# itailang/SampleNet

Hardware: NVIDIA H100
Metric: point-clouds/sec SampleNet fwd+Chamfer (B=32, N=1024->64) (higher is better)
Workload: dtype f32

## Files before the change

### samplenet_b200/csrc/conv_stack.cu

```cuda
#include "encoder_internal.cuh"
#include <cooperative_groups.h>
#include <string.h>

namespace snb {

constexpr int kCsMaxLayers = SNB200_MAX_CONV_LAYERS;
constexpr int kCsMaxSlicesPerCta = 32;
constexpr int kCsThreads = 512;
constexpr int kCsMaxPts = 128;
constexpr int kCsMinPts = 64;
constexpr int kCsNPT = kCsMaxPts / 4;
constexpr int kCsChunks = 4;
constexpr int kCsMaxSeg = 8;
constexpr int kCsLoPlane = kCsMaxPts * 128;
constexpr uint32_t kCsSlotBytes = 2u * kCsLoPlane;
constexpr int kCsWLd = 132;
constexpr uint32_t kCsWOff = kCsChunks * kCsSlotBytes;
constexpr uint32_t kCsAccOff = 2 * kCsSlotBytes;
constexpr size_t kCsSmemBytes = (size_t)kCsWOff + 128 * kCsWLd * sizeof(float) + 1024;

struct CsLayer {
    int c_in, c_out;
    const float *weight, *bias;
    const float *gamma, *beta, *run_mean, *run_var;
    float eps;
    int has_bn, relu;
    double *stats;
    float *zsave;
};

struct CsParams {
    const float *x; int layout;
    int b, n;
    long long total;
    int ppc, npt;
    int slots_per_cloud;
    int num_layers;
    CsLayer L[kCsMaxLayers];
    int training;
    double *mom;
    unsigned *barrier;
    float *tile_max, *tile_min;
    int fuse_head;
    HeadParams H;
    int self_clean;
    char *clean_ptr;
    unsigned clean_bytes;
    int slices_per_cta, num_slices;
    float *act[2];
    int act_ld;
    int head_rows;
};

__device__ __forceinline__ void cs_grid_arrive(unsigned *counter)
{
    asm volatile("red.release.gpu.global.add.u32 [%0], 1;" ::"l"(counter) : "memory");
}
__device__ __forceinline__ void cs_grid_wait(unsigned *counter, unsigned target)
{
    unsigned v, spin = 0;
    do {
        asm volatile("ld.acquire.gpu.global.u32 %0, [%1];" : "=r"(v) : "l"(counter) : "memory");
        if (++spin > (1u << 26)) __trap();
    } while (v < target);
}
__device__ __forceinline__ void cs_grid_barrier(unsigned *counter, unsigned target)
{
    __syncthreads();
    if (threadIdx.x == 0) {
        __threadfence();
        atomicAdd(counter, 1u);
        unsigned v, spin = 0;
        do {
            asm volatile("ld.acquire.gpu.global.u32 %0, [%1];" : "=r"(v) : "l"(counter) : "memory");
            if (++spin > (1u << 26)) __trap();
        } while (v < target);
    }
    __syncthreads();
}

__device__ __forceinline__ void cs_xchg_store(float *p, float v)
{
    unsigned u = __float_as_uint(v);
    if (u == 0u) u = 0x80000000u;
    asm volatile("st.volatile.global.u32 [%0], %1;" ::"l"(p), "r"(u) : "memory");
}
__device__ __forceinline__ unsigned cs_xchg_load1(const float *p)
{
    unsigned v;
    asm volatile("ld.volatile.global.u32 %0, [%1];" : "=r"(v) : "l"(p) : "memory");
    return v;
}
__device__ __forceinline__ uint4 cs_xchg_load4(const float *p)
{
    uint4 v;
    asm volatile("ld.volatile.global.v4.u32 {%0, %1, %2, %3}, [%4];" : "=r"(v.x), "=r"(v.y), "=r"(v.z), "=r"(v.w) : "l"(p) : "memory");
    return v;
}

__device__ __forceinline__ void cs_head_stage_weights(const HeadLayer &L, int cb, int nch, float *s_wh, int tid)
{
    const int c_in = L.c_in;
    if ((c_in & 3) == 0) {
        const int q4 = c_in >> 2, total = 8 * q4;
        for (int e0 = tid; e0 < total; e0 += kCsThreads * 4) {
            float4 v[4];
#pragma unroll
            for (int u = 0; u < 4; u++) {
                const int e = e0 + u * kCsThreads;
                const int jr = e / q4, kq = e - jr * q4;
                v[u] = (e < total && jr < nch) ? __ldg(reinterpret_cast<const float4 *>(L.weight + (size_t)(cb + jr) * c_in) + kq) : make_float4(0, 0, 0, 0);
            }
#pragma unroll
            for (int u = 0; u < 4; u++) {
                const int e = e0 + u * kCsThreads;
                if (e < total) *reinterpret_cast<float4 *>(s_wh + (size_t)e * 4) = v[u];
            }
        }
    } else {
        for (int e = tid; e < 8 * c_in; e += kCsThreads) {
            const int jr = e / c_in, k = e - jr * c_in;
            s_wh[e] = (jr < nch) ? __ldg(L.weight + (size_t)(cb + jr) * c_in + k) : 0.f;
        }
    }
}


__device__ __forceinline__ float cs_ld_now(const float *p)
{
    float v;
    asm volatile("ld.global.cg.f32 %0, [%1];" : "=f"(v) : "l"(p) : "memory");
    return v;
}

template <int KR>
__device__ __forceinline__ void cs_head_dot(const float *x, const float *w, int c_in, float (&a4)[4])
{
    float xr[KR];
#pragma unroll
    for (int i = 0; i < KR; i++) xr[i] = x[i];
#pragma unroll
    for (int i = 0; i < KR; i += 4) {
#pragma unroll
        for (int j = 0; j < 4; j++) {
            const float4 wv = *reinterpret_cast<const float4 *>(w + j * c_in + i);
            a4[j] = fmaf(xr[i + 3], wv.w, fmaf(xr[i + 2], wv.z, fmaf(xr[i + 1], wv.y, fmaf(xr[i], wv.x, a4[j]))));
        }
    }
}

__device__ __forceinline__ double cs_stat(const double *base, int c2, int idx, int spread)
{
    return __ldcg(spread ? base + c2 + (size_t)idx * kStatStride : base + idx);
}

constexpr unsigned long long kFxCountOne = 1ull << 56, kFxFieldMask = kFxCountOne - 1;
constexpr long long kFxSumOffset = 1ll << 47;
__device__ __forceinline__ unsigned long long *cs_fx_line(double *stats, int C, int idx)
{
    return reinterpret_cast<unsigned long long *>(stats + 2 * C + (size_t)idx * kStatStride);
}
__device__ __forceinline__ void cs_fx_add(unsigned long long *p, unsigned long long v)
{
    asm volatile("red.relaxed.gpu.global.add.u64 [%0], %1;" ::"l"(p), "l"(v) : "memory");
}
__device__ __forceinline__ unsigned long long cs_fx_load(const unsigned long long *p)
{
    unsigned long long v;
    asm volatile("ld.relaxed.gpu.global.u64 %0, [%1];" : "=l"(v) : "l"(p) : "memory");
    return v;
}
__device__ __forceinline__ bool cs_fx_contribute(double *stats, int C, int ch, float sum, float sumsq)
{
    const bool ok = fabsf(sum) < 8388608.f && sumsq < 274877906944.f;
    if (!ok) { sum = 0.f; sumsq = 0.f; }
    const long long ps = __double2ll_rn((double)sum * 16777216.0) + kFxSumOffset;
    const double qd = (double)sumsq, qh = floor(qd * 512.0);
    const long long hi = (long long)qh, lo = __double2ll_rn((qd - qh * (1.0 / 512.0)) * 281474976710656.0);
    unsigned long long *la = cs_fx_line(stats, C, ch), *lb = cs_fx_line(stats, C, C + ch);
    cs_fx_add(la, kFxCountOne + (unsigned long long)ps);
    cs_fx_add(lb, kFxCountOne + (unsigned long long)hi);
    cs_fx_add(la + 1, kFxCountOne + (unsigned long long)lo);
    return ok;
}
__device__ __forceinline__ void cs_fx_collect(double *stats, int C, int ch, unsigned G, double &sum, double &sumsq)
{
    const unsigned long long *la = cs_fx_line(stats, C, ch), *lb = cs_fx_line(stats, C, C + ch);
    unsigned long long a, b, c;
    unsigned spin = 0;
    do {
        a = cs_fx_load(la); c = cs_fx_load(la + 1); b = cs_fx_load(lb);
        if (++spin > (1u << 24)) __trap();
    } while ((unsigned)(a >> 56) != G || (unsigned)(b >> 56) != G || (unsigned)(c >> 56) != G);
    sum = (double)((long long)(a & kFxFieldMask) - (long long)G * kFxSumOffset) * (1.0 / 16777216.0);
    sumsq = (double)(long long)(b & kFxFieldMask) * (1.0 / 512.0) + (double)(long long)(c & kFxFieldMask) * (1.0 / 281474976710656.0);
}

__device__ __forceinline__ void cs_named_sync(int id, int nthreads) { asm volatile("bar.sync %0, %1;" ::"r"(id), "r"(nthreads) : "memory"); }

#ifdef SNB200_CS_TIMELINE
constexpr int kCsTlMaxCtas = 256, kCsTlMaxSlices = 8;
constexpr int kCsTlPerLayer = 2 + 5 * kCsTlMaxSlices;
constexpr int kCsTlHead = 2 + (kCsMaxLayers - 1) * kCsTlPerLayer, kCsTlStamps = kCsTlHead + 2;
__device__ unsigned long long g_cs_tl[kCsTlMaxCtas][kCsTlStamps][2];
__device__ __forceinline__ int cs_tl_layer(int l) { return 2 + (l - 1) * kCsTlPerLayer; }
__device__ __forceinline__ void cs_tl_stamp(int idx)
{
    if (threadIdx.x == 0 && blockIdx.x < kCsTlMaxCtas && idx >= 0 && idx < kCsTlStamps) {
        unsigned long long c, t;
        asm volatile("mov.u64 %0, %%clock64;" : "=l"(c) :: "memory");
        asm volatile("mov.u64 %0, %%globaltimer;" : "=l"(t) :: "memory");
        g_cs_tl[blockIdx.x][idx][0] = c;
        g_cs_tl[blockIdx.x][idx][1] = t;
    }
}
#define CS_TL(idx) cs_tl_stamp(idx)
#define CS_TL_SLICE(l, t, k) do { if ((t) < kCsTlMaxSlices) cs_tl_stamp(cs_tl_layer(l) + 1 + 5 * (t) + (k)); } while (0)
#else
#define CS_TL(idx) do { } while (0)
#define CS_TL_SLICE(l, t, k) do { } while (0)
#endif

__device__ __forceinline__ void cs_copy_w(float *sW, const CsLayer &L, int ch, int g, uint64_t *bar)
{
    const int K = L.c_in, N = L.c_out;
    if (ch < N) {
        if (g == 0) {
            fence_proxy_async();
            if (ch == 0) mbar_expect_tx(bar, (uint32_t)(N * K) * 4u);
            tma_load_1d(sW + (size_t)ch * kCsWLd, L.weight + (size_t)ch * K, (uint32_t)K * 4u, bar);
        }
    } else {
        float4 *z = reinterpret_cast<float4 *>(sW + (size_t)ch * kCsWLd + g * (K >> 2));
#pragma unroll
        for (int i = 0; i < 8; i++)
            if (i * 16 < K) z[i] = make_float4(0.f, 0.f, 0.f, 0.f);
    }
}
__device__ __forceinline__ void cs_wait_w(uint64_t *bar, int c) { mbar_wait(bar, (uint32_t)c & 1u); }

__device__ __forceinline__ void cs_wg_wait_1() { asm volatile("wgmma.wait_group.sync.aligned 1;" ::: "memory"); }

__device__ __forceinline__ void cs_write_chunk(const uint32_t (&v)[kCsNPT], float sc, float sh, float floor_v, int npt, uint32_t base, uint32_t gsw)
{
#pragma unroll
    for (int jb = 0; jb < kCsNPT / 8; jb++) {
        if (jb * 8 < npt) {
#pragma unroll
            for (int i = 0; i < 8; i++) {
                const float t = fmaxf(fmaf(__uint_as_float(v[jb * 8 + i]), sc, sh), floor_v);
                const float h = tf32_hi(t);
                const uint32_t a = base + (gsw ^ (uint32_t)(i << 4)) + (uint32_t)(jb * 1024 + i * 128);
                asm volatile("st.shared.f32 [%0], %1;" ::"r"(a), "f"(h) : "memory");
                asm volatile("st.shared.f32 [%0], %1;" ::"r"(a + (uint32_t)kCsLoPlane), "f"(t - h) : "memory");
            }
        }
    }
}

__device__ __forceinline__ int cs_acc_idx(int pt, int ch) { return pt * 128 + (ch ^ (((pt >> 1) & 3) << 3)); }

__device__ __forceinline__ void cs_save_rows(float *dst, int ld, const uint32_t (&v)[kCsNPT], int nvalid)
{
#pragma unroll
    for (int j = 0; j < kCsNPT; j++)
        if (j < nvalid) dst[j * ld] = __uint_as_float(v[j]);
}

__device__ __forceinline__ void cs_load_rows(const float *src, int ld, uint32_t (&v)[kCsNPT], int nvalid)
{
#pragma unroll
    for (int j = 0; j < kCsNPT; j++) v[j] = (j < nvalid) ? __float_as_uint(__ldcg(src + j * ld)) : 0u;
}

template <bool kMulti>
__global__ void __launch_bounds__(kCsThreads, 1) conv_stack_kernel(const __grid_constant__ CsParams P)
{
    extern __shared__ __align__(1024) unsigned char smem_raw[];
    __shared__ __align__(16) float sX[kCsMaxPts * 3];
    __shared__ float sW1[128 * 3], sB1[128];
    __shared__ float sRedS[4][128], sRedQ[4][128];
    __shared__ double sMom[9];
    __shared__ float sMomW[kCsThreads / 32][9];
    __shared__ int sBad;
    __shared__ uint64_t sWbar;

    const int tid = threadIdx.x, warp = tid >> 5, lane = tid & 31;
    const int q = warp & 3, g = (warp >> 2) & 3;
    const int ch = q * 32 + lane;
    const int G = gridDim.x;
    const int ppc = P.ppc, npt = P.npt, n = P.n;
    const long long P0 = (long long)blockIdx.x * ppc;
    const int npts = (int)min((long long)ppc, P.total - P0);
    const int col0 = g * npt;
    const int nvalid = max(0, min(npt, npts - col0));
    unsigned char *smem = smem_raw + ((1024u - (smem_u32(smem_raw) & 1023u)) & 1023u);
    float *sW = reinterpret_cast<float *>(smem + kCsWOff);
    float *sAcc = reinterpret_cast<float *>(smem + kCsAccOff);
    CS_TL(0);

    if (tid < 9) sMom[tid] = 0.0;
    if (tid == 0) sBad = 0;
    if (warp == 1) {
        if (lane == 0) mbar_init(&sWbar, 1);
        fence_mbar_init();
    }
    const CsLayer &L1 = P.L[0];
    const int nslices = kMulti ? (P.num_slices - (int)blockIdx.x + G - 1) / G : 1;
    auto load_x_slice = [&](const long long P0s, const int nptss) {
        if (P.layout == SNB200_BNC) {
            const float *src = P.x + P0s * 3;
            const int nf = nptss * 3;
            for (int e = tid; e < ppc * 3; e += kCsThreads) sX[e] = (e < nf) ? __ldg(src + e) : 0.f;
        } else {
            for (int e = tid; e < ppc * 3; e += kCsThreads) {
                const int c = e / ppc, r = e - c * ppc;
                float xv = 0.f;
                if (r < nptss) {
                    const int gp = (int)P0s + r;
                    const int cloud = gp / n, pi = gp - cloud * n;
                    xv = __ldg(P.x + ((size_t)cloud * 3 + c) * n + pi);
                }
                sX[r * 3 + c] = xv;
            }
        }
    };
    if (!kMulti) load_x_slice(P0, npts);
    for (int e = tid; e < L1.c_out * 3; e += kCsThreads) sW1[e] = __ldg(L1.weight + e);
    for (int e = tid; e < L1.c_out; e += kCsThreads) sB1[e] = L1.bias ? __ldg(L1.bias + e) : 0.f;
    __syncthreads();
    unsigned barrier_epoch = 0;
    const bool need_stats = P.training != 0;
    if (P.self_clean) {
        float4 *z = reinterpret_cast<float4 *>(P.clean_ptr);
        const unsigned n16 = P.clean_bytes >> 4;
        for (unsigned e = blockIdx.x * kCsThreads + tid; e < n16; e += G * kCsThreads) z[e] = make_float4(0.f, 0.f, 0.f, 0.f);
        if (!(need_stats && L1.has_bn)) cs_grid_barrier(P.barrier, ++barrier_epoch * G);
    }

    cs_copy_w(sW, P.L[1], ch, g, &sWbar);

    if (need_stats && L1.has_bn) {
        const int mom_pts = kMulti ? ppc : npts;
        float a9[9] = {0, 0, 0, 0, 0, 0, 0, 0, 0};
        for (int t = 0; t < nslices; t++) {
            int nptss = npts;
            if (kMulti) {
                const long long P0s = (long long)((int)blockIdx.x + t * G) * ppc;
                nptss = (int)min((long long)ppc, P.total - P0s);
                __syncthreads();
                load_x_slice(P0s, nptss);
                __syncthreads();
            }
            if (tid < nptss) {
                const float px = sX[tid * 3 + 0], py = sX[tid * 3 + 1], pz = sX[tid * 3 + 2];
                a9[0] += px; a9[1] += py; a9[2] += pz;
                a9[3] = fmaf(px, px, a9[3]); a9[4] = fmaf(px, py, a9[4]); a9[5] = fmaf(px, pz, a9[5]);
                a9[6] = fmaf(py, py, a9[6]); a9[7] = fmaf(py, pz, a9[7]); a9[8] = fmaf(pz, pz, a9[8]);
            }
        }
        if (warp * 32 < mom_pts) {
#pragma unroll
            for (int j = 0; j < 9; j++) {
                float v = a9[j];
                for (int o = 16; o > 0; o >>= 1) v += __shfl_xor_sync(kFullMask, v, o);
                if (lane == 0) sMomW[warp][j] = v;
            }
        }
        __syncthreads();
        if (tid < 9) {
            double t = 0.0;
            for (int w = 0; w * 32 < mom_pts && w < kCsThreads / 32; w++) t += (double)sMomW[w][tid];
            atomicAdd(P.mom + tid, t);
            cs_grid_arrive(reinterpret_cast<unsigned *>(P.mom + 9));
        }
    }
    if (need_stats && L1.has_bn) {
        if (tid < 9) {
            cs_grid_wait(reinterpret_cast<unsigned *>(P.mom + 9), 9u * G);
            sMom[tid] = __ldcg(P.mom + tid);
        }
        __syncthreads();
    }
    CS_TL(1);

    uint32_t v[kCsNPT];
    auto layer1_eval = [&](const long long P0s, const int nvalids) {
        if (q * 32 < L1.c_out) {
            const bool cv = ch < L1.c_out;
            const float w0 = cv ? sW1[ch * 3 + 0] : 0.f, w1 = cv ? sW1[ch * 3 + 1] : 0.f, w2 = cv ? sW1[ch * 3 + 2] : 0.f, b1 = cv ? sB1[ch] : 0.f;
#pragma unroll
            for (int jb = 0; jb < kCsNPT / 8; jb++) {
                if (jb * 8 < npt) {
                    const float4 *xq = reinterpret_cast<const float4 *>(sX + (col0 + jb * 8) * 3);
                    float xr[24];
#pragma unroll
                    for (int u = 0; u < 6; u++) { const float4 t4 = xq[u]; xr[u * 4 + 0] = t4.x; xr[u * 4 + 1] = t4.y; xr[u * 4 + 2] = t4.z; xr[u * 4 + 3] = t4.w; }
#pragma unroll
                    for (int i = 0; i < 8; i++) v[jb * 8 + i] = __float_as_uint(fmaf(w2, xr[i * 3 + 2], fmaf(w1, xr[i * 3 + 1], w0 * xr[i * 3 + 0])) + b1);
                }
            }
            if (L1.zsave && cv) cs_save_rows(L1.zsave + ((int)P0s + col0) * L1.c_out + ch, L1.c_out, v, nvalids);
        }
    };
    if (!kMulti) layer1_eval(P0, nvalid);

    for (int l = 1; l < P.num_layers; l++) {
        const CsLayer &Lp = P.L[l - 1];
        const CsLayer &Lc = P.L[l];
        const int K = Lc.c_in, N = Lc.c_out;
        const int nchunks = K >> 5;
        const bool last = (l == P.num_layers - 1);
        const bool want_stats = need_stats && Lc.has_bn;

        {
            float sc = 1.f, sh = 0.f;
            if (Lp.has_bn && ch < K && g == 0) {
                const float pgamma = cs_ld_now(Lp.gamma + ch), pbeta = cs_ld_now(Lp.beta + ch);

                float mean, var;
                if (P.training) {
                    const double cnt = (double)P.total, inv_cnt = 1.0 / cnt;
                    double m, vv;
                    if (l == 1) {
                        const double mx = sMom[0] * inv_cnt, my = sMom[1] * inv_cnt, mz = sMom[2] * inv_cnt;
                        const double cxx = sMom[3] * inv_cnt - mx * mx, cxy = sMom[4] * inv_cnt - mx * my, cxz = sMom[5] * inv_cnt - mx * mz;
                        const double cyy = sMom[6] * inv_cnt - my * my, cyz = sMom[7] * inv_cnt - my * mz, czz = sMom[8] * inv_cnt - mz * mz;
                        const double a0 = sW1[ch * 3 + 0], a1 = sW1[ch * 3 + 1], a2 = sW1[ch * 3 + 2];
                        m = a0 * mx + a1 * my + a2 * mz + (double)sB1[ch];
                        vv = a0 * a0 * cxx + a1 * a1 * cyy + a2 * a2 * czz + 2.0 * (a0 * a1 * cxy + a0 * a2 * cxz + a1 * a2 * cyz);
                        if (vv < 0) vv = 0;
                        if (blockIdx.x == 0) {
                            Lp.stats[ch] = cnt * m;
                            Lp.stats[K + ch] = cnt * (vv + m * m);
                        }
                    } else {
                        double s1, s2;
                        cs_fx_collect(Lp.stats, K, ch, (unsigned)G, s1, s2);
                        if (blockIdx.x == 0) { Lp.stats[ch] = s1; Lp.stats[K + ch] = s2; }
                        m = s1 * inv_cnt;
                        vv = s2 * inv_cnt - m * m;
                        if (vv < 0) vv = 0;
                    }
                    mean = (float)m; var = (float)vv;
                } else {
                    mean = Lp.run_mean[ch]; var = Lp.run_var[ch];
                }
                const float invstd = 1.0f / sqrtf(var + Lp.eps);
                sc = pgamma * invstd;
                sh = pbeta - mean * sc;
            }
            if (Lp.has_bn) {
                if (g == 0 && ch < K) { sRedS[0][ch] = sc; sRedQ[0][ch] = sh; }
                cs_named_sync(1, kCsThreads);
                if (ch < K) { sc = sRedS[0][ch]; sh = sRedQ[0][ch]; }
                cs_named_sync(1, kCsThreads);
            }
            CS_TL(cs_tl_layer(l));
            const int mh = g & 1, nh = g >> 1;
            const bool mma_wg = mh * 64 < N && nh * 64 < ppc;
            const float bias = (ch < N && Lc.bias) ? __ldg(Lc.bias + ch) : 0.f;
            float sumL = 0.f, sqL = 0.f;
            const float *act_in = kMulti && l > 1 ? (Lp.zsave ? Lp.zsave : P.act[(l - 1) & 1]) : nullptr;
            float *act_out = kMulti && !last ? (Lc.zsave ? Lc.zsave : P.act[l & 1]) : Lc.zsave;
            const int ld_in = (kMulti && !Lp.zsave && P.act_ld) ? P.act_ld : K, ld_out = (kMulti && !last && !Lc.zsave && P.act_ld) ? P.act_ld : N;
            auto write_tiles = [&](const int sl, const int cl_first, const int nseg, const float *sPmax, const float *sPmin) {
                const int S = P.slots_per_cloud;
                for (int e = tid; e < nseg * N; e += kCsThreads) {
                    const int s = e / N, c = e - s * N;
                    const int cl = cl_first + s;
                    const int slot = sl - cl * n / ppc;
                    float mx = -INFINITY, mn = INFINITY;
#pragma unroll
                    for (int gg = 0; gg < 4; gg++) {
                        mx = fmaxf(mx, sPmax[(gg * kCsMaxSeg + s) * 128 + c]);
                        mn = fminf(mn, sPmin[(gg * kCsMaxSeg + s) * 128 + c]);
                    }
                    if (sBad) { mx = INFINITY; mn = -INFINITY; }
                    P.tile_max[((size_t)cl * S + slot) * N + c] = mx;
                    P.tile_min[((size_t)cl * S + slot) * N + c] = mn;
                    if (((cl + 1) * n - 1) / ppc == sl)
                        for (int s2 = slot + 1; s2 < S; s2++) {
                            P.tile_max[((size_t)cl * S + s2) * N + c] = -INFINITY;
                            P.tile_min[((size_t)cl * S + s2) * N + c] = INFINITY;
                        }
                }
            };
            int cl_first = 0, nseg = 0;
            float *sPmax = reinterpret_cast<float *>(smem);
            float *sPmin = sPmax + 4 * kCsMaxSeg * 128;
            for (int t = 0; t < nslices; t++) {
                const int sl = kMulti ? (int)blockIdx.x + t * G : (int)blockIdx.x;
                const long long P0 = (long long)sl * ppc;
                const int npts = (int)min((long long)ppc, P.total - P0);
                const int nvalid = max(0, min(npt, npts - col0));
                const bool lastslice = !kMulti || t == nslices - 1;
                if (kMulti) {
#pragma unroll
                    for (int j = 0; j < kCsNPT; j++) v[j] = 0u;
                    if (l == 1) {
                        __syncthreads();
                        load_x_slice(P0, npts);
                        __syncthreads();
                        layer1_eval(P0, nvalid);
                    } else if (ch < K) {
                        cs_load_rows(act_in + ((int)P0 + col0) * ld_in + ch, ld_in, v, nvalid);
                    }
                }
                CS_TL_SLICE(l, t, 0);
                if (q < nchunks) {
                    const uint32_t base = smem_u32(smem) + (uint32_t)q * kCsSlotBytes + (uint32_t)col0 * 128u + (uint32_t)((lane & 3) << 2);
                    cs_write_chunk(v, sc, sh, Lp.relu ? 0.f : -INFINITY, npt, base, (uint32_t)((lane >> 2) << 4));
                    fence_proxy_async();
                }
                if (t == 0 && tid == 0) cs_wait_w(&sWbar, l - 1);
                __syncthreads();
                CS_TL_SLICE(l, t, 1);
                float acc[32];
                if (mma_wg) {
#pragma unroll
                    for (int i = 0; i < 32; i++) acc[i] = 0.f;
                    const float *wrow = sW + (size_t)(mh * 64 + q * 16 + (lane >> 2)) * kCsWLd + (lane & 3);
                    const uint32_t bbase = smem_u32(smem) + (uint32_t)nh * 64u * 128u;
                    uint32_t ahi[2][4], alo[2][4];
#pragma unroll 1
                    for (int c = 0; c < nchunks; c++) {
                        const uint32_t sb = bbase + (uint32_t)c * kCsSlotBytes;
#pragma unroll
                        for (int ks = 0; ks < 4; ks++) {
                            float w[4];
#pragma unroll
                            for (int e = 0; e < 4; e++) w[e] = wrow[(e & 1) * 8 * kCsWLd + c * 32 + ks * 8 + (e >> 1) * 4];
                            cs_wg_wait_1();
#pragma unroll
                            for (int e = 0; e < 4; e++) {
                                const float h = tf32_hi(w[e]);
                                ahi[ks & 1][e] = __float_as_uint(h);
                                alo[ks & 1][e] = __float_as_uint(w[e] - h);
                            }
                            wg_fence();
                            const uint64_t b_hi = wg_sdesc(sb + (uint32_t)(ks * 32));
                            const uint64_t b_lo = wg_sdesc(sb + (uint32_t)(kCsLoPlane + ks * 32));
                            wg_mma_rs_n64(acc, alo[ks & 1], b_hi, (c > 0 || ks > 0) ? 1u : 0u);
                            wg_mma_rs_n64(acc, ahi[ks & 1], b_lo, 1u);
                            wg_mma_rs_n64(acc, ahi[ks & 1], b_hi, 1u);
                            wg_commit();
                        }
                    }
                    wg_wait_all();
                }
                CS_TL_SLICE(l, t, 2);
                __syncthreads();
                if (mma_wg) {
                    const int r0 = mh * 64 + q * 16 + (lane >> 2), cq = nh * 64 + 2 * (lane & 3);
                    float *st0 = sAcc + cs_acc_idx(cq, r0), *st8 = sAcc + cs_acc_idx(cq, r0 + 8);
#pragma unroll
                    for (int j = 0; j < 8; j++) {
                        st0[j * 1024] = acc[4 * j + 0];
                        st0[j * 1024 + 128] = acc[4 * j + 1];
                        st8[j * 1024] = acc[4 * j + 2];
                        st8[j * 1024 + 128] = acc[4 * j + 3];
                    }
                }
                __syncthreads();
                if (!last && lastslice) cs_copy_w(sW, P.L[l + 1], ch, g, &sWbar);
                cl_first = (int)P0 / n;
                nseg = ((int)P0 + npts - 1) / n - cl_first + 1;
#pragma unroll
                for (int j = 0; j < kCsNPT; j++) v[j] = __float_as_uint(sAcc[col0 * 128 + cs_acc_idx(j, ch)]);
                CS_TL_SLICE(l, t, 3);
                if (q * 32 < N) {
                    float sum = 0.f, sq = 0.f;
#pragma unroll
                    for (int j = 0; j < kCsNPT; j++) {
                        const float u = __uint_as_float(v[j]) + bias;
                        v[j] = __float_as_uint(u);
                        if (j < nvalid) { sum += u; sq = fmaf(u, u, sq); }
                    }
                    if (kMulti) { sumL += sum; sqL += sq; }
                    else if (want_stats) { sRedS[g][ch] = sum; sRedQ[g][ch] = sq; }
                    if (act_out && ch < N) cs_save_rows(act_out + ((int)P0 + col0) * ld_out + ch, ld_out, v, nvalid);
                    if (last) {
                        for (int sgi = 0; sgi < nseg; sgi++) { sPmax[(g * kCsMaxSeg + sgi) * 128 + ch] = -INFINITY; sPmin[(g * kCsMaxSeg + sgi) * 128 + ch] = INFINITY; }
                        const long long gp0 = P0 + col0;
                        const int cl = (int)gp0 / n;
                        const int first_nb = (int)((long long)(cl + 1) * n - gp0);
                        if (nvalid == npt && first_nb >= npt) {
                            float mx = -INFINITY, mn = INFINITY;
#pragma unroll
                            for (int jb = 0; jb < kCsNPT / 8; jb++) {
                                if (jb * 8 < npt) {
#pragma unroll
                                    for (int i = 0; i < 8; i++) { mx = fmaxf(mx, __uint_as_float(v[jb * 8 + i])); mn = fminf(mn, __uint_as_float(v[jb * 8 + i])); }
                                }
                            }
                            sPmax[(g * kCsMaxSeg + cl - cl_first) * 128 + ch] = mx; sPmin[(g * kCsMaxSeg + cl - cl_first) * 128 + ch] = mn;
                        } else {
                            int jlo = 0;
                            for (int c2 = cl; jlo < nvalid; c2++) {
                                const int jhi = min(nvalid, (int)((long long)(c2 + 1) * n - gp0));
                                float mx = -INFINITY, mn = INFINITY;
#pragma unroll
                                for (int j = 0; j < kCsNPT; j++) {
                                    const bool in = j >= jlo && j < jhi;
                                    mx = in ? fmaxf(mx, __uint_as_float(v[j])) : mx;
                                    mn = in ? fminf(mn, __uint_as_float(v[j])) : mn;
                                }
                                sPmax[(g * kCsMaxSeg + c2 - cl_first) * 128 + ch] = mx; sPmin[(g * kCsMaxSeg + c2 - cl_first) * 128 + ch] = mn;
                                jlo = jhi;
                            }
                        }
                    }
                }
                if (kMulti) {
                    cs_named_sync(1, kCsThreads);
                    if (last) {
                        write_tiles(sl, cl_first, nseg, sPmax, sPmin);
                        cs_named_sync(1, kCsThreads);
                    }
                }
                CS_TL_SLICE(l, t, 4);
            }
            if (kMulti && want_stats && q * 32 < N) { sRedS[g][ch] = sumL; sRedQ[g][ch] = sqL; }
            if (want_stats || last) cs_named_sync(1, kCsThreads);
            if (want_stats && g == 0 && ch < N) {
                const float sm = (sRedS[0][ch] + sRedS[1][ch]) + (sRedS[2][ch] + sRedS[3][ch]);
                const float sqq = (sRedQ[0][ch] + sRedQ[1][ch]) + (sRedQ[2][ch] + sRedQ[3][ch]);
                if (last) {
                    double *acc = Lc.stats + 2 * N;
                    atomicAdd(acc + (size_t)ch * kStatStride, (double)sm);
                    atomicAdd(acc + (size_t)(N + ch) * kStatStride, (double)sqq);
                } else if (!cs_fx_contribute(Lc.stats, N, ch, sm, sqq)) {
                    sBad = 1;
                }
            }
            if (last && !kMulti) write_tiles((int)blockIdx.x, cl_first, nseg, sPmax, sPmin);
            if (want_stats && last) {
                cs_named_sync(1, kCsThreads);
                if (tid == 0) {
                    cs_grid_arrive(P.barrier);
                    cs_grid_wait(P.barrier, (barrier_epoch + 1) * G);
                }
                cs_named_sync(1, kCsThreads);
            } else if (!last && !want_stats) {
                cs_named_sync(1, kCsThreads);
            }
            CS_TL(cs_tl_layer(l) + kCsTlPerLayer - 1);
        }
        if (want_stats && last) barrier_epoch++;
    }

    __syncthreads();
    CS_TL(kCsTlHead);

    asm volatile("griddepcontrol.launch_dependents;" ::: "memory");
    if (!P.fuse_head) {
        const CsLayer &LL = P.L[P.num_layers - 1];
        if (blockIdx.x == 0 && need_stats && LL.has_bn && tid < 2 * LL.c_out) LL.stats[tid] = cs_stat(LL.stats, 2 * LL.c_out, tid, 1);
        CS_TL(kCsTlHead + 1);
        return;
    }
    const HeadParams &H = P.H;
    float *s_in = reinterpret_cast<float *>(smem_raw);
    int hcmax = H.c_feat, hcsum = 0;
    for (int l = 0; l < H.num_fc; l++) { hcmax = max(hcmax, H.fc[l].c_in); hcsum += H.fc[l].c_in; }
    const int RS = P.head_rows, gpb = RS >> 5;
    float *s_part = reinterpret_cast<float *>(smem_raw) + (size_t)RS * (hcmax + 1);
    float *s_wall = s_part + 8 * 8 * 32;
    __shared__ uint64_t hbar[SNB200_MAX_FC_LAYERS];
    const double inv_cnt_h = 1.0 / H.count;
    const float inv_b = 1.0f / (float)H.b;
    if (tid == 0) {
        for (int l = 0; l < H.num_fc; l++) mbar_init(&hbar[l], 1);
        fence_mbar_init();
        fence_proxy_async();
        int woff = 0;
        for (int l = 0; l < H.num_fc; l++) {
            const HeadLayer &L = H.fc[l];
            const int cpc = max(8, (((L.c_out + G - 1) / G + 7) / 8) * 8);
            const int lo = blockIdx.x * cpc, hi = min(L.c_out, lo + cpc);
            const bool tma_ok = (L.c_in & 3) == 0 && (hcmax & 3) == 0 && (reinterpret_cast<uintptr_t>(L.weight) & 15) == 0;
            if (lo < hi && tma_ok) {
                const uint32_t bytes = (uint32_t)min(8, hi - lo) * L.c_in * 4u;
                mbar_expect_tx(&hbar[l], bytes);
                tma_load_1d(s_wall + woff, L.weight + (size_t)lo * L.c_in, bytes, &hbar[l]);
            }
            woff += 8 * L.c_in;
        }
    }
    if (!(need_stats && P.L[P.num_layers - 1].has_bn)) cs_grid_barrier(P.barrier, ++barrier_epoch * G);
    {
        const int total = H.b * H.c_feat;
        const int gt = (G - 1 - (int)blockIdx.x) * kCsThreads + tid, gn = G * kCsThreads;
        float *ll0 = H.ll[0];
        for (int e = gt; e < total; e += gn) {
            const int bi = e / H.c_feat, c = e % H.c_feat;
            float mx = -INFINITY, mn = INFINITY;
            const float *tm = H.tile_max + (size_t)bi * H.tiles_per_cloud * H.c_feat + c;
            const float *tn = H.tile_min + (size_t)bi * H.tiles_per_cloud * H.c_feat + c;
            const double st0 = (H.last_has_bn && H.training) ? cs_stat(H.last_stats, 2 * H.c_feat, c, H.stat_rep) : 0.0;
            const double st1 = (H.last_has_bn && H.training) ? cs_stat(H.last_stats, 2 * H.c_feat, H.c_feat + c, H.stat_rep) : 0.0;
            if (H.stat_rep && bi == 0 && H.last_has_bn && H.training) {
                double *canon = const_cast<double *>(H.last_stats);
                canon[c] = st0; canon[H.c_feat + c] = st1;
            }
            const float lg = H.last_has_bn ? __ldg(H.last_gamma + c) : 1.f, lb = H.last_has_bn ? __ldg(H.last_beta + c) : 0.f;
// ... 250 lines not shown
                P.barrier[1] = 0u;
            }
        }
    }
    CS_TL(kCsTlHead + 1);
}

struct CsPartition { int ppc, slices, grid, per_cta; };
static CsPartition cs_partition(long long total)
{
    const int sms = num_sms();
    const long long rounds = max(1ll, (total + (long long)sms * kCsMaxPts - 1) / ((long long)sms * kCsMaxPts));
    long long ppc = (total + sms * rounds - 1) / (sms * rounds);
    ppc = (ppc + 31) / 32 * 32;
    if (ppc < kCsMinPts) ppc = kCsMinPts;
    if (ppc > kCsMaxPts) ppc = kCsMaxPts;
    CsPartition R;
    R.ppc = (int)ppc;
    R.slices = (int)((total + ppc - 1) / ppc);
    R.grid = min(sms, R.slices);
    R.per_cta = (R.slices + R.grid - 1) / R.grid;
    return R;
}
static int cs_points_per_cta(long long total) { return cs_partition(total).ppc; }

void conv_stack_partition(int b, int n, int *ppc, int *slices, int *grid, int *per_cta, int *slots)
{
    const CsPartition R = cs_partition((long long)b * n);
    *ppc = R.ppc; *slices = R.slices; *grid = R.grid; *per_cta = R.per_cta;
    *slots = (n - 1) / R.ppc + 2;
}

int conv_stack_slots_per_cloud(int b, int n)
{
    const int ppc = cs_points_per_cta((long long)b * n);
    return (n - 1) / ppc + 2;
}

bool conv_stack_supported(int b, int n, int nconv, const snb200_layer *conv)
{
    if (nconv < 2 || nconv > kCsMaxLayers || conv[0].c_in != 3) return false;
    if (conv[0].c_out % 32 != 0 || conv[0].c_out > 128) return false;
    for (int l = 1; l < nconv; l++) {
        if ((conv[l].c_in != 32 && conv[l].c_in != 64 && conv[l].c_in != 128) || conv[l].c_out > 128 || conv[l].c_out < 8) return false;
        if (reinterpret_cast<uintptr_t>(conv[l].weight) & 15) return false;
    }
    const long long total = (long long)b * n;
    const CsPartition R = cs_partition(total);
    if (R.per_cta > kCsMaxSlicesPerCta) return false;
    if ((R.ppc - 1) / n + 2 > kCsMaxSeg) return false;
    if (R.grid > 255) return false;
    return true;
}

int launch_conv_stack(int b, int n, int layout, const float *x, int nconv, const snb200_layer *conv, int training, double *const *stats,
                      double *mom, unsigned *barrier, float *tile_max, float *tile_min, const HeadParams *head,
                      char *clean_ptr, size_t clean_bytes, cudaStream_t stream, float *const *zsave, float *const *act)
{
    CsParams P;
    memset(&P, 0, sizeof(P));
    if (head) { P.fuse_head = 1; P.H = *head; }
    if (head && clean_ptr) { P.self_clean = 1; P.clean_ptr = clean_ptr; P.clean_bytes = (unsigned)clean_bytes; }
    P.x = x; P.layout = layout; P.b = b; P.n = n;
    P.total = (long long)b * n;
    const CsPartition R = cs_partition(P.total);
    P.ppc = R.ppc; P.slices_per_cta = R.per_cta; P.num_slices = R.slices;
    const bool multi = R.per_cta > 1;
    if (multi && !(act && act[0] && act[1])) { set_error("conv stack: %d slices per CTA need the activation workspace", R.per_cta); return SNB200_EINVAL; }
    if (act) { P.act[0] = act[0]; P.act[1] = act[1]; }
    bool layers_ordered = training != 0;
    for (int l = 0; l < nconv; l++) layers_ordered = layers_ordered && conv[l].bn_weight != nullptr;
    P.act_ld = 0;
    if (!layers_ordered) { P.act_ld = 8; for (int l = 0; l + 1 < nconv; l++) P.act_ld = max(P.act_ld, conv[l].c_out); }
    P.npt = P.ppc / 4;
    P.slots_per_cloud = (n - 1) / P.ppc + 2;
    P.num_layers = nconv; P.training = training;
    P.mom = mom; P.barrier = barrier; P.tile_max = tile_max; P.tile_min = tile_min;
    for (int l = 0; l < nconv; l++) {
        CsLayer &D = P.L[l];
        D.c_in = conv[l].c_in; D.c_out = conv[l].c_out; D.weight = conv[l].weight; D.bias = conv[l].bias;
        D.gamma = conv[l].bn_weight; D.beta = conv[l].bn_bias; D.run_mean = conv[l].bn_running_mean; D.run_var = conv[l].bn_running_var;
        D.eps = conv[l].bn_eps; D.has_bn = conv[l].bn_weight != nullptr; D.relu = conv[l].relu; D.stats = stats[l];
        D.zsave = zsave ? zsave[l] : nullptr;
    }
    if (head) {
        P.H.tiles_per_cloud = P.slots_per_cloud;
        P.H.stat_rep = 1;
        for (int i = 0; i < P.H.ru_num; i++) P.H.ru_rep[i] = (P.H.ru_stats[i] == stats[nconv - 1]) ? 1 : 0;
    }
    size_t smem = kCsSmemBytes;
    if (head) {
        int hcmax = head->c_feat;
        for (int l = 0; l < head->num_fc; l++) hcmax = max(hcmax, head->fc[l].c_in);
        size_t hcsum = 0;
        for (int l = 0; l < head->num_fc; l++) hcsum += head->fc[l].c_in;
        int rs = min(128, (b + 31) / 32 * 32);
        size_t hs = 0;
        for (;; rs -= 32) {
            hs = ((size_t)rs * (hcmax + 1) + 2048 + (size_t)8 * hcsum) * sizeof(float) + 1024;
            if (hs <= 200 * 1024 || rs == 32) break;
        }
        if (hs > 200 * 1024) { set_error("conv stack: FC width %d too large for the fused head", hcmax); return SNB200_EUNSUPPORTED; }
        P.head_rows = rs;
        smem = max(smem, hs);
    }
    static PerDeviceOnce once;
    if (once.first()) {
        cudaFuncSetAttribute(conv_stack_kernel<false>, cudaFuncAttributeMaxDynamicSharedMemorySize, 204 * 1024);
        cudaFuncSetAttribute(conv_stack_kernel<true>, cudaFuncAttributeMaxDynamicSharedMemorySize, 204 * 1024);
    }
    const int grid = R.grid;
    cudaLaunchConfig_t cfg;
    memset(&cfg, 0, sizeof(cfg));
    cfg.gridDim = dim3(grid); cfg.blockDim = dim3(kCsThreads); cfg.dynamicSmemBytes = smem; cfg.stream = stream;
    cudaLaunchAttribute attr[1];
    attr[0].id = cudaLaunchAttributeCooperative;
    attr[0].val.cooperative = 1;
    cfg.attrs = attr; cfg.numAttrs = 1;
    cudaError_t e = multi ? cudaLaunchKernelEx(&cfg, conv_stack_kernel<true>, P) : cudaLaunchKernelEx(&cfg, conv_stack_kernel<false>, P);
    if (e != cudaSuccess) { set_error("conv stack: cooperative launch failed: %s", cudaGetErrorString(e)); cudaGetLastError(); return SNB200_ECUDA; }
    return check_launch("conv stack");
}

}

#ifdef SNB200_CS_TIMELINE
extern "C" __attribute__((visibility("default"))) int snb200_cs_timeline(unsigned long long *host, size_t bytes)
{
    void *dev = nullptr;
    if (bytes != sizeof(snb::g_cs_tl) || cudaDeviceSynchronize() != cudaSuccess) return -1;
    if (cudaMemcpyFromSymbol(host, snb::g_cs_tl, bytes) != cudaSuccess || cudaGetSymbolAddress(&dev, snb::g_cs_tl) != cudaSuccess) return -1;
    if (cudaMemset(dev, 0, bytes) != cudaSuccess || cudaDeviceSynchronize() != cudaSuccess) return -1;
    return snb::kCsTlStamps;
}
extern "C" __attribute__((visibility("default"))) int snb200_cs_timeline_layout(int *max_ctas, int *max_slices, int *per_layer, int *head)
{
    *max_ctas = snb::kCsTlMaxCtas; *max_slices = snb::kCsTlMaxSlices; *per_layer = snb::kCsTlPerLayer; *head = snb::kCsTlHead;
    return snb::kCsTlStamps;
}
#endif
```

Before: 248,100.

## Stage multi-slice input via cp.async and keep last slice in smem across layers

In the multi-slice cooperative path, the input points for up to eight slices are prefetched into shared memory with cp.async, so the per-slice global loads and barriers in the moment pass and in layer 1 go away. The slice order is also reordered so each layer starts with the slice held over from the previous layer. That slice's activations are read from the shared accumulator instead of global memory, and its store is skipped. Statistics accumulation is reworked through shared memory to match the new order. The cost is more dynamic shared memory and more complex ordering logic that could break the batch-norm statistics.

```diff
diff --git a/samplenet_b200/csrc/conv_stack.cu b/samplenet_b200/csrc/conv_stack.cu
--- a/samplenet_b200/csrc/conv_stack.cu
+++ b/samplenet_b200/csrc/conv_stack.cu
@@ -18,6 +18,9 @@
 constexpr uint32_t kCsWOff = kCsChunks * kCsSlotBytes;
 constexpr uint32_t kCsAccOff = 2 * kCsSlotBytes;
 constexpr size_t kCsSmemBytes = (size_t)kCsWOff + 128 * kCsWLd * sizeof(float) + 1024;
+constexpr int kCsXStageSlices = 8;
+constexpr uint32_t kCsXOff = kCsWOff + 128 * kCsWLd * sizeof(float);
+constexpr size_t kCsSmemBytesMulti = kCsSmemBytes + (size_t)kCsXStageSlices * kCsMaxPts * 3 * sizeof(float);
 
 struct CsLayer {
     int c_in, c_out;
@@ -132,6 +135,11 @@
     asm volatile("ld.global.cg.f32 %0, [%1];" : "=f"(v) : "l"(p) : "memory");
     return v;
 }
+__device__ __forceinline__ void cs_cp_async4(float *dst, const float *src)
+{
+    asm volatile("cp.async.ca.shared.global [%0], [%1], 4;" ::"r"(smem_u32(dst)), "l"(src) : "memory");
+}
+__device__ __forceinline__ void cs_cp_async_wait_all() { asm volatile("cp.async.wait_all;" ::: "memory"); }
 
 template <int KR>
 __device__ __forceinline__ void cs_head_dot(const float *x, const float *w, int c_in, float (&a4)[4])
@@ -283,6 +291,7 @@
     __shared__ double sMom[9];
     __shared__ float sMomW[kCsThreads / 32][9];
     __shared__ int sBad;
+    __shared__ float sHeld[2][kCsThreads];
     __shared__ uint64_t sWbar;
 
     const int tid = threadIdx.x, warp = tid >> 5, lane = tid & 31;
@@ -326,6 +335,25 @@
         }
     };
     if (!kMulti) load_x_slice(P0, npts);
+    const bool staged = kMulti && nslices <= kCsXStageSlices;
+    const float *sXs = reinterpret_cast<const float *>(smem + kCsXOff);
+    if (staged) {
+        float *dst = reinterpret_cast<float *>(smem + kCsXOff);
+        for (int e = tid; e < nslices * ppc * 3; e += kCsThreads) {
+            const int t = e / (ppc * 3), et = e - t * (ppc * 3);
+            const int P0s = ((int)blockIdx.x + t * G) * ppc;
+            const int nptss = (int)min((long long)ppc, P.total - P0s);
+            const int c = P.layout == SNB200_BNC ? et % 3 : et / ppc, r = P.layout == SNB200_BNC ? et / 3 : et - c * ppc;
+            float *d = dst + t * (kCsMaxPts * 3) + r * 3 + c;
+            if (r >= nptss) {
+                *d = 0.f;
+            } else {
+                const int gp = P0s + r;
+                const int cloud = gp / n, pi = gp - cloud * n;
+                cs_cp_async4(d, P.layout == SNB200_BNC ? P.x + (size_t)gp * 3 + c : P.x + ((size_t)cloud * 3 + c) * n + pi);
+            }
+        }
+    }
     for (int e = tid; e < L1.c_out * 3; e += kCsThreads) sW1[e] = __ldg(L1.weight + e);
     for (int e = tid; e < L1.c_out; e += kCsThreads) sB1[e] = L1.bias ? __ldg(L1.bias + e) : 0.f;
     __syncthreads();
@@ -339,21 +367,30 @@
     }
 
     cs_copy_w(sW, P.L[1], ch, g, &sWbar);
+    if (staged) {
+        cs_cp_async_wait_all();
+        __syncthreads();
+    }
 
     if (need_stats && L1.has_bn) {
         const int mom_pts = kMulti ? ppc : npts;
         float a9[9] = {0, 0, 0, 0, 0, 0, 0, 0, 0};
         for (int t = 0; t < nslices; t++) {
             int nptss = npts;
+            const float *xs = sX;
             if (kMulti) {
                 const long long P0s = (long long)((int)blockIdx.x + t * G) * ppc;
                 nptss = (int)min((long long)ppc, P.total - P0s);
-                __syncthreads();
-                load_x_slice(P0s, nptss);
-                __syncthreads();
+                if (staged) {
+                    xs = sXs + t * (kCsMaxPts * 3);
+                } else {
+                    __syncthreads();
+                    load_x_slice(P0s, nptss);
+                    __syncthreads();
+                }
             }
             if (tid < nptss) {
-                const float px = sX[tid * 3 + 0], py = sX[tid * 3 + 1], pz = sX[tid * 3 + 2];
+                const float px = xs[tid * 3 + 0], py = xs[tid * 3 + 1], pz = xs[tid * 3 + 2];
                 a9[0] += px; a9[1] += py; a9[2] += pz;
                 a9[3] = fmaf(px, px, a9[3]); a9[4] = fmaf(px, py, a9[4]); a9[5] = fmaf(px, pz, a9[5]);
                 a9[6] = fmaf(py, py, a9[6]); a9[7] = fmaf(py, pz, a9[7]); a9[8] = fmaf(pz, pz, a9[8]);
@@ -385,14 +422,14 @@
     CS_TL(1);
 
     uint32_t v[kCsNPT];
-    auto layer1_eval = [&](const long long P0s, const int nvalids) {
+    auto layer1_eval = [&](const long long P0s, const int nvalids, const float *xs) {
         if (q * 32 < L1.c_out) {
             const bool cv = ch < L1.c_out;
             const float w0 = cv ? sW1[ch * 3 + 0] : 0.f, w1 = cv ? sW1[ch * 3 + 1] : 0.f, w2 = cv ? sW1[ch * 3 + 2] : 0.f, b1 = cv ? sB1[ch] : 0.f;
 #pragma unroll
             for (int jb = 0; jb < kCsNPT / 8; jb++) {
                 if (jb * 8 < npt) {
-                    const float4 *xq = reinterpret_cast<const float4 *>(sX + (col0 + jb * 8) * 3);
+                    const float4 *xq = reinterpret_cast<const float4 *>(xs + (col0 + jb * 8) * 3);
                     float xr[24];
 #pragma unroll
                     for (int u = 0; u < 6; u++) { const float4 t4 = xq[u]; xr[u * 4 + 0] = t4.x; xr[u * 4 + 1] = t4.y; xr[u * 4 + 2] = t4.z; xr[u * 4 + 3] = t4.w; }
@@ -403,7 +440,7 @@
             if (L1.zsave && cv) cs_save_rows(L1.zsave + ((int)P0s + col0) * L1.c_out + ch, L1.c_out, v, nvalids);
         }
     };
-    if (!kMulti) layer1_eval(P0, nvalid);
+    if (!kMulti) layer1_eval(P0, nvalid, sX);
 
     for (int l = 1; l < P.num_layers; l++) {
         const CsLayer &Lp = P.L[l - 1];
@@ -412,7 +449,9 @@
         const int nchunks = K >> 5;
         const bool last = (l == P.num_layers - 1);
         const bool want_stats = need_stats && Lc.has_bn;
-
+        const int held = l == 1 ? -1 : (nslices == 1 || (l & 1) == 0) ? nslices - 1 : nslices - 2;
+
+        const float pbias = (kMulti && l > 1 && ch < K && Lp.bias) ? cs_ld_now(Lp.bias + ch) : 0.f;
         {
             float sc = 1.f, sh = 0.f;
             if (Lp.has_bn && ch < K && g == 0) {
@@ -460,7 +499,6 @@
             const int mh = g & 1, nh = g >> 1;
             const bool mma_wg = mh * 64 < N && nh * 64 < ppc;
             const float bias = (ch < N && Lc.bias) ? __ldg(Lc.bias + ch) : 0.f;
-            float sumL = 0.f, sqL = 0.f;
             const float *act_in = kMulti && l > 1 ? (Lp.zsave ? Lp.zsave : P.act[(l - 1) & 1]) : nullptr;
             float *act_out = kMulti && !last ? (Lc.zsave ? Lc.zsave : P.act[l & 1]) : Lc.zsave;
             const int ld_in = (kMulti && !Lp.zsave && P.act_ld) ? P.act_ld : K, ld_out = (kMulti && !last && !Lc.zsave && P.act_ld) ? P.act_ld : N;
@@ -489,8 +527,10 @@
             int cl_first = 0, nseg = 0;
             float *sPmax = reinterpret_cast<float *>(smem);
             float *sPmin = sPmax + 4 * kCsMaxSeg * 128;
+            if (kMulti && want_stats && q * 32 < N) { sRedS[g][ch] = 0.f; sRedQ[g][ch] = 0.f; }
             for (int t = 0; t < nslices; t++) {
-                const int sl = kMulti ? (int)blockIdx.x + t * G : (int)blockIdx.x;
+                const int u = !kMulti ? 0 : held < 0 ? t : t == 0 ? held : (t - 1 < held ? t - 1 : t);
+                const int sl = kMulti ? (int)blockIdx.x + u * G : (int)blockIdx.x;
                 const long long P0 = (long long)sl * ppc;
                 const int npts = (int)min((long long)ppc, P.total - P0);
                 const int nvalid = max(0, min(npt, npts - col0));
@@ -499,10 +539,20 @@
 #pragma unroll
                     for (int j = 0; j < kCsNPT; j++) v[j] = 0u;
                     if (l == 1) {
-                        __syncthreads();
-                        load_x_slice(P0, npts);
-                        __syncthreads();
-                        layer1_eval(P0, nvalid);
+                        if (staged) {
+                            layer1_eval(P0, nvalid, sXs + u * (kCsMaxPts * 3));
+                        } else {
+                            __syncthreads();
+                            load_x_slice(P0, npts);
+                            __syncthreads();
+                            layer1_eval(P0, nvalid, sX);
+                        }
+                    } else if (t == 0) {
+                        const int nheld = ch < K ? nvalid : 0;
+#pragma unroll
+                        for (int j = 0; j < kCsNPT; j++)
+                            if (j < nheld) v[j] = __float_as_uint(sAcc[col0 * 128 + cs_acc_idx(j, ch)] + pbias);
+                        cs_named_sync(1, kCsThreads);
                     } else if (ch < K) {
                         cs_load_rows(act_in + ((int)P0 + col0) * ld_in + ch, ld_in, v, nvalid);
                     }
@@ -577,9 +627,16 @@
                         v[j] = __float_as_uint(u);
                         if (j < nvalid) { sum += u; sq = fmaf(u, u, sq); }
                     }
-                    if (kMulti) { sumL += sum; sqL += sq; }
-                    else if (want_stats) { sRedS[g][ch] = sum; sRedQ[g][ch] = sq; }
-                    if (act_out && ch < N) cs_save_rows(act_out + ((int)P0 + col0) * ld_out + ch, ld_out, v, nvalid);
+                    if (kMulti) {
+                        if (t == 0 && held >= 0) {
+                            sHeld[0][tid] = sum; sHeld[1][tid] = sq;
+                        } else if (want_stats) {
+                            float s = sRedS[g][ch], s2 = sRedQ[g][ch];
+                            if (held >= 0 && u == held + 1) { s += sHeld[0][tid]; s2 += sHeld[1][tid]; }
+                            sRedS[g][ch] = s + sum; sRedQ[g][ch] = s2 + sq;
+                        }
+                    } else if (want_stats) { sRedS[g][ch] = sum; sRedQ[g][ch] = sq; }
+                    if (act_out && (!kMulti || Lc.zsave || !lastslice) && ch < N) cs_save_rows(act_out + ((int)P0 + col0) * ld_out + ch, ld_out, v, nvalid);
                     if (last) {
                         for (int sgi = 0; sgi < nseg; sgi++) { sPmax[(g * kCsMaxSeg + sgi) * 128 + ch] = -INFINITY; sPmin[(g * kCsMaxSeg + sgi) * 128 + ch] = INFINITY; }
                         const long long gp0 = P0 + col0;
@@ -621,7 +678,7 @@
                 }
                 CS_TL_SLICE(l, t, 4);
             }
-            if (kMulti && want_stats && q * 32 < N) { sRedS[g][ch] = sumL; sRedQ[g][ch] = sqL; }
+            if (kMulti && want_stats && q * 32 < N && held == nslices - 1) { sRedS[g][ch] += sHeld[0][tid]; sRedQ[g][ch] += sHeld[1][tid]; }
             if (want_stats || last) cs_named_sync(1, kCsThreads);
             if (want_stats && g == 0 && ch < N) {
                 const float sm = (sRedS[0][ch] + sRedS[1][ch]) + (sRedS[2][ch] + sRedS[3][ch]);
@@ -1044,7 +1101,7 @@
         P.H.stat_rep = 1;
         for (int i = 0; i < P.H.ru_num; i++) P.H.ru_rep[i] = (P.H.ru_stats[i] == stats[nconv - 1]) ? 1 : 0;
     }
-    size_t smem = kCsSmemBytes;
+    size_t smem = multi ? kCsSmemBytesMulti : kCsSmemBytes;
     if (head) {
         int hcmax = head->c_feat;
         for (int l = 0; l < head->num_fc; l++) hcmax = max(hcmax, head->fc[l].c_in);
@@ -1063,7 +1120,7 @@
     static PerDeviceOnce once;
     if (once.first()) {
         cudaFuncSetAttribute(conv_stack_kernel<false>, cudaFuncAttributeMaxDynamicSharedMemorySize, 204 * 1024);
-        cudaFuncSetAttribute(conv_stack_kernel<true>, cudaFuncAttributeMaxDynamicSharedMemorySize, 204 * 1024);
+        cudaFuncSetAttribute(conv_stack_kernel<true>, cudaFuncAttributeMaxDynamicSharedMemorySize, (int)kCsSmemBytesMulti);
     }
     const int grid = R.grid;
     cudaLaunchConfig_t cfg;
```

Result: faster. 258,400 (median of 6 runs) (+4.1%).

## Prefetch next slice activations into shared memory via TMA bulk loads

Applied to the files above, without the earlier changes.

In the multi-slice conv stack path, inter-layer activation rows for the next slice are fetched with a 1D TMA bulk copy into shared memory, signalled by a new mbarrier. The current slice's GEMM runs while that copy is in flight. The layer's first slice is issued at the end of the previous layer, after an async-proxy fence on the global writes. When K<=64, the accumulator staging is moved to the base shared region so the prefetch buffer does not collide with it. This hides global-load latency of the per-column __ldcg reads, at the cost of extra barriers, phase tracking and shared-memory aliasing risk.

```diff
diff --git a/samplenet_b200/csrc/conv_stack.cu b/samplenet_b200/csrc/conv_stack.cu
--- a/samplenet_b200/csrc/conv_stack.cu
+++ b/samplenet_b200/csrc/conv_stack.cu
@@ -273,6 +273,21 @@
     for (int j = 0; j < kCsNPT; j++) v[j] = (j < nvalid) ? __float_as_uint(__ldcg(src + j * ld)) : 0u;
 }
 
+__device__ __forceinline__ void cs_read_rows(const float *src, int ld, uint32_t (&v)[kCsNPT], int nvalid)
+{
+#pragma unroll
+    for (int j = 0; j < kCsNPT; j++) v[j] = (j < nvalid) ? __float_as_uint(src[j * ld]) : 0u;
+}
+
+__device__ __forceinline__ void cs_fence_parked() { asm volatile("fence.proxy.async.global;" ::: "memory"); }
+
+__device__ __forceinline__ void cs_fetch_rows(float *dst, const float *src, uint32_t bytes, uint64_t *bar)
+{
+    fence_proxy_async();
+    mbar_expect_tx(bar, bytes);
+    tma_load_1d(dst, src, bytes, bar);
+}
+
 template <bool kMulti>
 __global__ void __launch_bounds__(kCsThreads, 1) conv_stack_kernel(const __grid_constant__ CsParams P)
 {
@@ -284,6 +299,7 @@
     __shared__ float sMomW[kCsThreads / 32][9];
     __shared__ int sBad;
     __shared__ uint64_t sWbar;
+    __shared__ uint64_t sRbar;
 
     const int tid = threadIdx.x, warp = tid >> 5, lane = tid & 31;
     const int q = warp & 3, g = (warp >> 2) & 3;
@@ -303,6 +319,7 @@
     if (tid == 0) sBad = 0;
     if (warp == 1) {
         if (lane == 0) mbar_init(&sWbar, 1);
+        if (kMulti && lane == 0) mbar_init(&sRbar, 1);
         fence_mbar_init();
     }
     const CsLayer &L1 = P.L[0];
@@ -404,6 +421,7 @@
         }
     };
     if (!kMulti) layer1_eval(P0, nvalid);
+    unsigned rows_phase = 0;
 
     for (int l = 1; l < P.num_layers; l++) {
         const CsLayer &Lp = P.L[l - 1];
@@ -464,6 +482,15 @@
             const float *act_in = kMulti && l > 1 ? (Lp.zsave ? Lp.zsave : P.act[(l - 1) & 1]) : nullptr;
             float *act_out = kMulti && !last ? (Lc.zsave ? Lc.zsave : P.act[l & 1]) : Lc.zsave;
             const int ld_in = (kMulti && !Lp.zsave && P.act_ld) ? P.act_ld : K, ld_out = (kMulti && !last && !Lc.zsave && P.act_ld) ? P.act_ld : N;
+            const bool rows_free = kMulti && K <= 64 && !last;
+            const bool rows_ok = kMulti && l > 1 && (reinterpret_cast<uintptr_t>(act_in) & 15) == 0;
+            const bool next_ok = kMulti && !last && (reinterpret_cast<uintptr_t>(act_out) & 15) == 0;
+            float *sRows = reinterpret_cast<float *>(smem + kCsAccOff);
+            float *sAccL = rows_free ? reinterpret_cast<float *>(smem) : sAcc;
+            auto fetch_next = [&](const int sl) {
+                const int P0n = (sl + G) * ppc;
+                cs_fetch_rows(sRows, act_in + P0n * ld_in, (uint32_t)(min(ppc, (int)P.total - P0n) * ld_in) * 4u, &sRbar);
+            };
             auto write_tiles = [&](const int sl, const int cl_first, const int nseg, const float *sPmax, const float *sPmin) {
                 const int S = P.slots_per_cloud;
                 for (int e = tid; e < nseg * N; e += kCsThreads) {
@@ -503,6 +530,12 @@
                         load_x_slice(P0, npts);
                         __syncthreads();
                         layer1_eval(P0, nvalid);
+                    } else if (rows_ok) {
+                        if (ch < K) {
+                            mbar_wait(&sRbar, (rows_phase + (unsigned)t) & 1u);
+                            cs_read_rows(sRows + col0 * ld_in + ch, ld_in, v, nvalid);
+                        }
+                        if (nchunks > 2) __syncthreads();
                     } else if (ch < K) {
                         cs_load_rows(act_in + ((int)P0 + col0) * ld_in + ch, ld_in, v, nvalid);
                     }
@@ -515,6 +548,7 @@
                 }
                 if (t == 0 && tid == 0) cs_wait_w(&sWbar, l - 1);
                 __syncthreads();
+                if (rows_ok && rows_free && !lastslice && tid == 0) fetch_next(sl);
                 CS_TL_SLICE(l, t, 1);
                 float acc[32];
                 if (mma_wg) {
@@ -553,7 +587,7 @@
                 __syncthreads();
                 if (mma_wg) {
                     const int r0 = mh * 64 + q * 16 + (lane >> 2), cq = nh * 64 + 2 * (lane & 3);
-                    float *st0 = sAcc + cs_acc_idx(cq, r0), *st8 = sAcc + cs_acc_idx(cq, r0 + 8);
+                    float *st0 = sAccL + cs_acc_idx(cq, r0), *st8 = sAccL + cs_acc_idx(cq, r0 + 8);
 #pragma unroll
                     for (int j = 0; j < 8; j++) {
                         st0[j * 1024] = acc[4 * j + 0];
@@ -567,7 +601,11 @@
                 cl_first = (int)P0 / n;
                 nseg = ((int)P0 + npts - 1) / n - cl_first + 1;
 #pragma unroll
-                for (int j = 0; j < kCsNPT; j++) v[j] = __float_as_uint(sAcc[col0 * 128 + cs_acc_idx(j, ch)]);
+                for (int j = 0; j < kCsNPT; j++) v[j] = __float_as_uint(sAccL[col0 * 128 + cs_acc_idx(j, ch)]);
+                if (rows_ok && !rows_free && !lastslice) {
+                    cs_named_sync(1, kCsThreads);
+                    if (tid == 0) fetch_next(sl);
+                }
                 CS_TL_SLICE(l, t, 3);
                 if (q * 32 < N) {
                     float sum = 0.f, sq = 0.f;
@@ -579,7 +617,10 @@
                     }
                     if (kMulti) { sumL += sum; sqL += sq; }
                     else if (want_stats) { sRedS[g][ch] = sum; sRedQ[g][ch] = sq; }
-                    if (act_out && ch < N) cs_save_rows(act_out + ((int)P0 + col0) * ld_out + ch, ld_out, v, nvalid);
+                    if (act_out && ch < N) {
+                        cs_save_rows(act_out + ((int)P0 + col0) * ld_out + ch, ld_out, v, nvalid);
+                        if (next_ok && lastslice) cs_fence_parked();
+                    }
                     if (last) {
                         for (int sgi = 0; sgi < nseg; sgi++) { sPmax[(g * kCsMaxSeg + sgi) * 128 + ch] = -INFINITY; sPmin[(g * kCsMaxSeg + sgi) * 128 + ch] = INFINITY; }
                         const long long gp0 = P0 + col0;
@@ -617,10 +658,14 @@
                     if (last) {
                         write_tiles(sl, cl_first, nseg, sPmax, sPmin);
                         cs_named_sync(1, kCsThreads);
+                    } else if (next_ok && lastslice && tid == 0) {
+                        const int P0f = (int)blockIdx.x * ppc;
+                        cs_fetch_rows(sRows, act_out + P0f * ld_out, (uint32_t)(min(ppc, (int)P.total - P0f) * ld_out) * 4u, &sRbar);
                     }
                 }
                 CS_TL_SLICE(l, t, 4);
             }
+            if (rows_ok) rows_phase += (unsigned)nslices;
             if (kMulti && want_stats && q * 32 < N) { sRedS[g][ch] = sumL; sRedQ[g][ch] = sqL; }
             if (want_stats || last) cs_named_sync(1, kCsThreads);
             if (want_stats && g == 0 && ch < N) {
```

Result: faster. 250,500 before, 254,300 after, median of 6 (+1.5%).

## Keep boundary slices on-chip across layers via alternating slice order

Applied to the files above, without the earlier changes.

In the multi-slice-per-CTA path, slice traversal order now reverses on odd layers. The last slice(s) processed in one layer become the first in the next, so their activations are kept in shared memory (accumulator buffer or spare weight-tile columns) instead of being written to and reread from the global activation workspace. A per-layer 'keep' count set on the host controls how many slices stay resident: up to two when channels are at most 64, otherwise one. This cuts global traffic and load latency at layer boundaries, at the cost of more complex indexing and reuse of the weight smem region, which could race with the next weight copy.

```diff
diff --git a/samplenet_b200/csrc/conv_stack.cu b/samplenet_b200/csrc/conv_stack.cu
--- a/samplenet_b200/csrc/conv_stack.cu
+++ b/samplenet_b200/csrc/conv_stack.cu
@@ -27,6 +27,7 @@
     int has_bn, relu;
     double *stats;
     float *zsave;
+    int keep;
 };
 
 struct CsParams {
@@ -196,6 +197,12 @@
     sumsq = (double)(long long)(b & kFxFieldMask) * (1.0 / 512.0) + (double)(long long)(c & kFxFieldMask) * (1.0 / 281474976710656.0);
 }
 
+__device__ __forceinline__ int cs_nctaid()
+{
+    int v;
+    asm volatile("mov.u32 %0, %%nctaid.x;" : "=r"(v));
+    return v;
+}
 __device__ __forceinline__ void cs_named_sync(int id, int nthreads) { asm volatile("bar.sync %0, %1;" ::"r"(id), "r"(nthreads) : "memory"); }
 
 #ifdef SNB200_CS_TIMELINE
@@ -490,21 +497,37 @@
             float *sPmax = reinterpret_cast<float *>(smem);
             float *sPmin = sPmax + 4 * kCsMaxSeg * 128;
             for (int t = 0; t < nslices; t++) {
-                const int sl = kMulti ? (int)blockIdx.x + t * G : (int)blockIdx.x;
+                const int tv = kMulti && (l & 1) ? nslices - 1 - t : t;
+                const int sl = kMulti ? (int)blockIdx.x + tv * cs_nctaid() : (int)blockIdx.x;
                 const long long P0 = (long long)sl * ppc;
                 const int npts = (int)min((long long)ppc, P.total - P0);
                 const int nvalid = max(0, min(npt, npts - col0));
                 const bool lastslice = !kMulti || t == nslices - 1;
+                const bool kept = kMulti && nslices - 1 - t < Lc.keep;
                 if (kMulti) {
 #pragma unroll
                     for (int j = 0; j < kCsNPT; j++) v[j] = 0u;
+                    const bool on_chip = t < Lp.keep;
                     if (l == 1) {
-                        __syncthreads();
-                        load_x_slice(P0, npts);
-                        __syncthreads();
+                        if (!on_chip) {
+                            __syncthreads();
+                            load_x_slice(P0, npts);
+                            __syncthreads();
+                        }
                         layer1_eval(P0, nvalid);
+                    } else if (on_chip && t == 0) {
+                        const float pbias = (ch < K && Lp.bias) ? __ldg(Lp.bias + ch) : 0.f;
+#pragma unroll
+                        for (int j = 0; j < kCsNPT; j++) v[j] = __float_as_uint(sAcc[col0 * 128 + cs_acc_idx(j, ch)] + pbias);
+                        if (nchunks > 2) __syncthreads();
                     } else if (ch < K) {
-                        cs_load_rows(act_in + ((int)P0 + col0) * ld_in + ch, ld_in, v, nvalid);
+                        if (on_chip) {
+                            const float *src = sW + col0 * kCsWLd + 64 + ch;
+#pragma unroll
+                            for (int j = 0; j < kCsNPT; j++) v[j] = (j < nvalid) ? __float_as_uint(src[j * kCsWLd]) : 0u;
+                        } else {
+                            cs_load_rows(act_in + ((int)P0 + col0) * ld_in + ch, ld_in, v, nvalid);
+                        }
                     }
                 }
                 CS_TL_SLICE(l, t, 0);
@@ -512,6 +535,11 @@
                     const uint32_t base = smem_u32(smem) + (uint32_t)q * kCsSlotBytes + (uint32_t)col0 * 128u + (uint32_t)((lane & 3) << 2);
                     cs_write_chunk(v, sc, sh, Lp.relu ? 0.f : -INFINITY, npt, base, (uint32_t)((lane >> 2) << 4));
                     fence_proxy_async();
+                }
+                if (kMulti && lastslice && t > 0 && Lc.keep >= 2 && ch < N) {
+#pragma unroll
+                    for (int j = 0; j < kCsNPT; j++) v[j] = __float_as_uint(sAcc[col0 * 128 + cs_acc_idx(j, ch)] + bias);
+                    cs_save_rows(sW + col0 * kCsWLd + 64 + ch, kCsWLd, v, npt);
                 }
                 if (t == 0 && tid == 0) cs_wait_w(&sWbar, l - 1);
                 __syncthreads();
@@ -579,7 +607,7 @@
                     }
                     if (kMulti) { sumL += sum; sqL += sq; }
                     else if (want_stats) { sRedS[g][ch] = sum; sRedQ[g][ch] = sq; }
-                    if (act_out && ch < N) cs_save_rows(act_out + ((int)P0 + col0) * ld_out + ch, ld_out, v, nvalid);
+                    if (act_out && ch < N && (Lc.zsave || !kept)) cs_save_rows(act_out + ((int)P0 + col0) * ld_out + ch, ld_out, v, nvalid);
                     if (last) {
                         for (int sgi = 0; sgi < nseg; sgi++) { sPmax[(g * kCsMaxSeg + sgi) * 128 + ch] = -INFINITY; sPmin[(g * kCsMaxSeg + sgi) * 128 + ch] = INFINITY; }
                         const long long gp0 = P0 + col0;
@@ -1038,6 +1066,9 @@
         D.gamma = conv[l].bn_weight; D.beta = conv[l].bn_bias; D.run_mean = conv[l].bn_running_mean; D.run_var = conv[l].bn_running_var;
         D.eps = conv[l].bn_eps; D.has_bn = conv[l].bn_weight != nullptr; D.relu = conv[l].relu; D.stats = stats[l];
         D.zsave = zsave ? zsave[l] : nullptr;
+        if (!multi || l == nconv - 1) D.keep = 0;
+        else if (l == 0) D.keep = (training && D.has_bn) ? 1 : 0;
+        else D.keep = (D.c_in <= 64 && D.c_out <= 64) ? 2 : 1;
     }
     if (head) {
         P.H.tiles_per_cloud = P.slots_per_cloud;
```

New measurement: 244,600 before, 275,900 after (median of 6 runs). 12.8% higher.
